# lucidrains/e2-tts-pytorch

Measured on NVIDIA H100. Metric: mel-frames/sec E2TTS fwd+bwd (d512 depth8 L1024), higher is better.
Workload: dtype bf16

## Files before the change

### e2-tts-pytorch_b200/csrc/gemm.cu

```cuda
#include <stdlib.h>

#include "common.cuh"
#include "ptx.cuh"

namespace b200 {

constexpr int BM = 128;
constexpr int BK = 64;
constexpr int kGemmThreads = 384;
constexpr int A_STAGE_BYTES = BM * BK * 2;
constexpr int kSliceBytes = 64 * 64 * 2;

struct GemmParams {
    int M, N, K;
    int tiles_m, tiles_n, num_work;
    int kb_total, kb_per_split, kb_a1;
    void* D; long long ldd; int d_fp32;
    void* D2; long long ldd2;
    const float* bias;
    const float* colscale; int rows_per_batch;
    const unsigned char* rowmask;
    const void* resid; long long ldr;
    int geglu; float dropout_p; unsigned long long seed;
    const unsigned long long* seed_dev;
    int atomic_out;
    int tma_store;
    int resid_tma;
    const float* glu_mult;
};

constexpr int GLU_GELU = 1, GLU_SILU = 2, GLU_RELU2 = 3;
constexpr int ACT_GELU = 1;

template <int BN, int MH>
struct GemmSmem {
    static constexpr int A_BYTES = MH * A_STAGE_BYTES;
    static constexpr int B_STAGE_BYTES = BN * BK * 2;
    static constexpr int STAGE_BYTES = A_BYTES + B_STAGE_BYTES;
    static constexpr int kStages = (STAGE_BYTES <= 32768) ? 6 : 4;
    static constexpr int TILE_BYTES = kStages * STAGE_BYTES;
    static constexpr int STG_BYTES = 2 * 2 * kSliceBytes;
    static constexpr int BAR_BYTES = 128;
    static_assert((2 * kStages + 4) * 8 <= BAR_BYTES, "GEMM mbarriers exceed their shared-memory slot");
    static constexpr int TOTAL = TILE_BYTES + STG_BYTES + BAR_BYTES + 1024;
    static_assert(TOTAL <= 227 * 1024, "GEMM shared memory exceeds the 227 KB a block may use");
};

__device__ __forceinline__ float2 gelu_erf2(float2 x) {
    const float2 a = make_float2(fabsf(x.x), fabsf(x.y));
    float2 t = ffma2(a, make_float2(-1.9449223600531695e-06f, -1.9449223600531695e-06f), make_float2(6.386057066265494e-05f, 6.386057066265494e-05f));
    t = ffma2(t, a, make_float2(-0.0009488713694736362f, -0.0009488713694736362f));
    t = ffma2(t, a, make_float2(0.008582375012338161f, 0.008582375012338161f));
    t = ffma2(t, a, make_float2(-0.0541183240711689f, -0.0541183240711689f));
    t = ffma2(t, a, make_float2(-0.4582974314689636f, -0.4582974314689636f));
    t = ffma2(t, a, make_float2(-1.1513246297836304f, -1.1513246297836304f));
    t = ffma2(t, a, make_float2(-0.9999869465827942f, -0.9999869465827942f));
    float ex, ey;
    asm("ex2.approx.ftz.f32 %0, %1;" : "=f"(ex) : "f"(t.x));
    asm("ex2.approx.ftz.f32 %0, %1;" : "=f"(ey) : "f"(t.y));
    return ffma2(make_float2(-a.x, -a.y), make_float2(ex, ey), make_float2(fmaxf(x.x, 0.f), fmaxf(x.y, 0.f)));
}

__device__ __forceinline__ float2 silu2(float2 x) {
    const float2 t = fmul2(x, make_float2(-1.4426950408889634f, -1.4426950408889634f));
    float ex, ey;
    asm("ex2.approx.ftz.f32 %0, %1;" : "=f"(ex) : "f"(t.x));
    asm("ex2.approx.ftz.f32 %0, %1;" : "=f"(ey) : "f"(t.y));
    const float2 d = fadd2(make_float2(ex, ey), make_float2(1.f, 1.f));
    return make_float2(__fdividef(x.x, d.x), __fdividef(x.y, d.y));
}

__device__ __forceinline__ float2 relu2_2(float2 x) {
    const float2 r = make_float2(fmaxf(x.x, 0.f), fmaxf(x.y, 0.f));
    return fmul2(r, r);
}

template <int ACT>
__device__ __forceinline__ float2 glu_act2(float2 g) {
    if constexpr (ACT == GLU_GELU) return gelu_erf2(g);
    else if constexpr (ACT == GLU_SILU) return silu2(g);
    else return relu2_2(g);
}

__device__ __forceinline__ uint32_t slice_addr(uint32_t buf, uint32_t toff, uint32_t swz, int i, int jj) {
    return buf + toff + (uint32_t)i * 8 * 128 + (((uint32_t)jj << 4) ^ swz);
}
__device__ __forceinline__ uint32_t slice_acquire(uint8_t* my_stg, uint32_t n, int cw, int t) {
    if (t == 0) bulk_wait_group_read<1>();
    named_bar_sync(1 + cw, 128);
    return smem_u32(my_stg + (n & 1) * kSliceBytes);
}
__device__ __forceinline__ void resid_load(const CUtensorMap* m, uint8_t* my_stg, uint64_t* my_rbar, uint32_t b, int c0, int c1) {
    mbar_arrive_expect_tx(&my_rbar[b], kSliceBytes);
    tma_load_2d(my_stg + b * kSliceBytes, m, &my_rbar[b], c0, c1);
}
__device__ __forceinline__ void slice_store(const CUtensorMap* m, uint8_t* my_stg, uint32_t n, int cw, int t, int c0, int c1) {
    fence_proxy_async();
    named_bar_sync(1 + cw, 128);
    if (t == 0) {
        tma_store_2d(m, my_stg + (n & 1) * kSliceBytes, c0, c1);
        bulk_commit_group();
    }
}

template <int ACT, int BN, int MH>
__device__ __forceinline__ void glu_epilogue(const GemmParams& p, float (&acc)[MH][BN / 2], int tm, int tn, int cw, int wq, int lane) {
    constexpr int BMT = BM * MH;
    const int cq = 2 * (lane & 3);
    const bool do_drop = p.dropout_p > 0.f;
    const float keep_scale = do_drop ? 65536.f / (65536.f - (float)(uint32_t)(p.dropout_p * 65536.f)) : 1.f;
    const uint32_t seedmix = do_drop ? seed_mix32(p.seed + (p.seed_dev ? __ldg(p.seed_dev) : 0ull)) : 0u;
    const uint32_t thr32 = drop_thresh32((uint32_t)(p.dropout_p * 65536.f));
#pragma unroll
    for (int h = 0; h < MH; ++h) {
#pragma unroll
        for (int i = 0; i < 2; ++i) {
            const int row = tm * BMT + (cw * MH + h) * 64 + wq * 16 + (lane >> 2) + 8 * i;
            if (row >= p.M) continue;
#pragma unroll
            for (int sub = 0; sub < BN / 128; ++sub) {
                const int colg = tn * BN + sub * 128;
                if (colg >= p.N) continue;
#pragma unroll
                for (int j = 0; j < 8; ++j) {
                    const int cu = colg + 8 * j + cq;
                    const int hcol = colg / 2 + 8 * j + cq;
                    float2 u = make_float2(acc[h][4 * (sub * 16 + j) + 2 * i], acc[h][4 * (sub * 16 + j) + 2 * i + 1]);
                    float2 g = make_float2(acc[h][4 * (sub * 16 + 8 + j) + 2 * i], acc[h][4 * (sub * 16 + 8 + j) + 2 * i + 1]);
                    if (p.bias) {
                        u = fadd2(u, make_float2(__ldg(p.bias + cu), __ldg(p.bias + cu + 1)));
                        g = fadd2(g, make_float2(__ldg(p.bias + cu + 64), __ldg(p.bias + cu + 65)));
                    }
                    const uint32_t wu = pack_bf16(u.x, u.y), wgt = pack_bf16(g.x, g.y);
                    if (p.D2) {
                        __nv_bfloat16* d2 = reinterpret_cast<__nv_bfloat16*>(p.D2) + (long long)row * p.ldd2 + cu;
                        *reinterpret_cast<uint32_t*>(d2) = wu;
                        *reinterpret_cast<uint32_t*>(d2 + 64) = wgt;
                    }
                    float2 h2 = fmul2(make_float2(bf16_lo(wu), bf16_hi(wu)), glu_act2<ACT>(make_float2(bf16_lo(wgt), bf16_hi(wgt))));
                    if (p.glu_mult) h2 = fmul2(h2, make_float2(__ldg(p.glu_mult + hcol), __ldg(p.glu_mult + hcol + 1)));
                    if (do_drop) {
                        const DropWords hsh = drop_words(seedmix, (uint32_t)(((unsigned long long)row * (unsigned long long)(p.N / 2) + hcol) >> 1));
                        h2 = fmul2(h2, make_float2(hsh.a >= thr32 ? keep_scale : 0.f, hsh.b >= thr32 ? keep_scale : 0.f));
                    }
                    *reinterpret_cast<uint32_t*>(reinterpret_cast<__nv_bfloat16*>(p.D) + (long long)row * p.ldd + hcol) = pack_bf16(h2.x, h2.y);
                }
            }
        }
    }
}


template <bool RESID, int BN, int MH>
__device__ __forceinline__ void store_slices(const GemmParams& p, float (&acc)[MH][BN / 2], const CUtensorMap* tmD, const CUtensorMap* tmR,
                                             uint8_t* my_stg, uint64_t* my_rbar, uint32_t& nslice, int tm, int tn, int cw, int wq, int lane,
                                             int t) {
    const uint32_t swz = (uint32_t)(lane >> 2) << 4;
    const uint32_t toff = (uint32_t)(wq * 16 + (lane >> 2)) * 128 + 4 * (lane & 3);
#pragma unroll
    for (int h = 0; h < MH; ++h) {
        const int rowb = tm * BM * MH + (cw * MH + h) * 64;
#pragma unroll
        for (int s = 0; s < BN / 64; ++s) {
            const int colb = tn * BN + s * 64;
            if (colb >= p.N) break;
            uint32_t buf;
            if constexpr (RESID) {
                buf = smem_u32(my_stg + (nslice & 1) * kSliceBytes);
                mbar_wait(&my_rbar[nslice & 1], (nslice >> 1) & 1);
            } else {
                buf = slice_acquire(my_stg, nslice, cw, t);
            }
#pragma unroll
            for (int i = 0; i < 2; ++i) {
#pragma unroll
                for (int jj = 0; jj < 8; ++jj) {
                    const int j = s * 8 + jj;
                    const uint32_t a = slice_addr(buf, toff, swz, i, jj);
                    float v0 = acc[h][4 * j + 2 * i], v1 = acc[h][4 * j + 2 * i + 1];
                    if constexpr (RESID) {
                        const uint32_t r = ld_shared_u32(a);
                        v0 += bf16_lo(r); v1 += bf16_hi(r);
                    }
                    st_shared_u32(a, pack_bf16(v0, v1));
                }
            }
            slice_store(tmD, my_stg, nslice, cw, t, colb, rowb);
            if constexpr (RESID) {
                const bool more = MH == 1 ? (s + 2 < BN / 64 && colb + 128 < p.N) : (h + 1 < MH && tn * BN + 64 < p.N);
                if (t == 0 && more) {
                    bulk_wait_group_read<0>();
                    resid_load(tmR, my_stg, my_rbar, nslice & 1, MH == 1 ? colb + 128 : colb, MH == 1 ? rowb : rowb + 64);
                }
            }
            ++nslice;
        }
    }
}

__device__ __forceinline__ void store_pair(const GemmParams& p, int row, int col, float v0, float v1) {
    const bool two = col + 1 < p.N;
    if (p.d_fp32) {
        float* dp = reinterpret_cast<float*>(p.D) + (long long)row * p.ldd + col;
        const bool vec = two && (reinterpret_cast<uintptr_t>(dp) & 7) == 0;
        if (p.atomic_out) {
            if (vec) atomicAdd(reinterpret_cast<float2*>(dp), make_float2(v0, v1));
            else { atomicAdd(dp, v0); if (two) atomicAdd(dp + 1, v1); }
        } else {
            if (vec) *reinterpret_cast<float2*>(dp) = make_float2(v0, v1);
            else { dp[0] = v0; if (two) dp[1] = v1; }
        }
    } else {
        __nv_bfloat16* dp = reinterpret_cast<__nv_bfloat16*>(p.D) + (long long)row * p.ldd + col;
        if (two) *reinterpret_cast<uint32_t*>(dp) = pack_bf16(v0, v1);
        else dp[0] = __float2bfloat16_rn(v0);
    }
}

template <int BN, bool A_MN, bool B_MN, int MH, int ACT>
__global__ void __launch_bounds__(kGemmThreads, 1)
gemm_wgmma_kernel(const __grid_constant__ CUtensorMap tmA, const __grid_constant__ CUtensorMap tmA2,
                  const __grid_constant__ CUtensorMap tmB, const __grid_constant__ CUtensorMap tmD,
                  const __grid_constant__ CUtensorMap tmR, const GemmParams p) {
    using S = GemmSmem<BN, MH>;
    constexpr int kStages = S::kStages;
    constexpr int BMT = BM * MH;
    constexpr int NACC = BN / 2;
    extern __shared__ uint8_t smem_raw[];
    uint8_t* smem = smem_raw + ((1024u - (smem_u32(smem_raw) & 1023u)) & 1023u);
    uint8_t* smA = smem;
    uint8_t* smB = smem + kStages * S::A_BYTES;
    uint8_t* stg = smem + S::TILE_BYTES;
    uint64_t* full_bar = reinterpret_cast<uint64_t*>(smem + S::TILE_BYTES + S::STG_BYTES);
    uint64_t* empty_bar = full_bar + kStages;
    uint64_t* resid_bar = empty_bar + kStages;

    const int wg = threadIdx.x >> 7;

    if (threadIdx.x == 0) {
        tma_prefetch_desc(&tmA);
        tma_prefetch_desc(&tmA2);
        tma_prefetch_desc(&tmB);
        if (p.tma_store) tma_prefetch_desc(&tmD);
        if (p.resid_tma) tma_prefetch_desc(&tmR);
        for (int i = 0; i < kStages; ++i) {
            mbar_init(&full_bar[i], 1);
            mbar_init(&empty_bar[i], 2);
        }
        for (int i = 0; i < 4; ++i) mbar_init(&resid_bar[i], 1);
        fence_barrier_init();
    }
    __syncthreads();

    if (wg == 0) {
        regs_dealloc<40>();
        if (threadIdx.x == 0) {
            int stage = 0;
            uint32_t phase = 0;
            for (int w = blockIdx.x; w < p.num_work; w += gridDim.x) {
                const int tm = w % p.tiles_m;
                const int rest = w / p.tiles_m;
                const int tn = rest % p.tiles_n;
                const int sp = rest / p.tiles_n;
                const int kb0 = sp * p.kb_per_split;
                const int kb1 = min(p.kb_total, kb0 + p.kb_per_split);
                const int arow = tm * BMT;
                const int brow = tn * BN;
                for (int kb = kb0; kb < kb1; ++kb) {
                    mbar_wait(&empty_bar[stage], phase ^ 1);
                    mbar_arrive_expect_tx(&full_bar[stage], S::STAGE_BYTES);
                    uint8_t* a_dst = smA + stage * S::A_BYTES;
                    uint8_t* b_dst = smB + stage * S::B_STAGE_BYTES;
                    const CUtensorMap* ma = kb < p.kb_a1 ? &tmA : &tmA2;
                    const int ka = kb < p.kb_a1 ? kb * BK : (kb - p.kb_a1) * BK;
                    if constexpr (!A_MN) {
#pragma unroll
                        for (int h = 0; h < MH; ++h) tma_load_2d(a_dst + h * A_STAGE_BYTES, ma, &full_bar[stage], ka, arow + h * BM);
                    } else {
#pragma unroll
                        for (int i = 0; i < BMT / 64; ++i) tma_load_2d(a_dst + i * (BK * 128), ma, &full_bar[stage], arow + i * 64, ka);
                    }
                    if constexpr (!B_MN) {
#pragma unroll
                        for (int h = 0; h < BN / 128; ++h) tma_load_2d(b_dst + h * (128 * BK * 2), &tmB, &full_bar[stage], kb * BK, brow + h * 128);
                    } else {
#pragma unroll
                        for (int i = 0; i < BN / 64; ++i) tma_load_2d(b_dst + i * (BK * 128), &tmB, &full_bar[stage], brow + i * 64, kb * BK);
                    }
                    if (++stage == kStages) { stage = 0; phase ^= 1; }
                }
            }
        }
        return;
    }

    regs_alloc<232>();
    const int cw = wg - 1;
    const int t = threadIdx.x & 127;
    const int lane = t & 31, wq = t >> 5;
    constexpr uint32_t a_lbo = A_MN ? BK * 128 : 16, b_lbo = B_MN ? BK * 128 : 16;
    constexpr uint32_t a_adv = A_MN ? (16 * 128) >> 4 : (16 * 2) >> 4;
    constexpr uint32_t b_adv = B_MN ? (16 * 128) >> 4 : (16 * 2) >> 4;
    float acc[MH][NACC];
    uint8_t* my_stg = stg + cw * 2 * kSliceBytes;
    uint64_t* my_rbar = resid_bar + cw * 2;
    uint32_t nslice = 0;
    int stage = 0;
    uint32_t phase = 0;
    for (int w = blockIdx.x; w < p.num_work; w += gridDim.x) {
        const int tm = w % p.tiles_m;
        const int rest = w / p.tiles_m;
        const int tn = rest % p.tiles_n;
        const int sp = rest / p.tiles_n;
        const int kb0 = sp * p.kb_per_split;
        const int kb1 = min(p.kb_total, kb0 + p.kb_per_split);
        const int kb_resid = max(kb0, kb1 - 2);
        int prev = -1;
        for (int kb = kb0; kb < kb1; ++kb) {
            mbar_wait(&full_bar[stage], phase);
#pragma unroll
            for (int h = 0; h < MH; ++h) fence_regs(acc[h]);
            wgmma_fence();
            const uint64_t bdesc = make_smem_desc_sw128(smem_u32(smB + stage * S::B_STAGE_BYTES), b_lbo, 1024);
#pragma unroll
            for (int h = 0; h < MH; ++h) {
                const uint64_t adesc = make_smem_desc_sw128(smem_u32(smA + stage * S::A_BYTES + (cw * MH + h) * 8192), a_lbo, 1024);
#pragma unroll
                for (int k = 0; k < BK / 16; ++k) {
                    const uint32_t accum = (kb > kb0 || k > 0) ? 1u : 0u;
                    if constexpr (BN == 256) wgmma_ss_n256<A_MN, B_MN>(acc[h], adesc + (uint64_t)(k * a_adv), bdesc + (uint64_t)(k * b_adv), accum);
                    else wgmma_ss_n128<A_MN, B_MN>(acc[h], adesc + (uint64_t)(k * a_adv), bdesc + (uint64_t)(k * b_adv), accum);
                }
            }
            wgmma_commit();
            if (p.resid_tma && kb == kb_resid && t == 0) {
                const int r0 = tm * BMT + cw * MH * 64;
                bulk_wait_group_read<0>();
                resid_load(&tmR, my_stg, my_rbar, nslice & 1, tn * BN, r0);
                if (tn * BN + 64 < p.N) resid_load(&tmR, my_stg, my_rbar, (nslice + 1) & 1, tn * BN + 64, r0);
                else if (MH == 2) resid_load(&tmR, my_stg, my_rbar, (nslice + 1) & 1, tn * BN, r0 + 64);
            }
            wgmma_wait<1>();
#pragma unroll
            for (int h = 0; h < MH; ++h) fence_regs(acc[h]);
            if (prev >= 0 && t == 0) mbar_arrive(&empty_bar[prev]);
            prev = stage;
            if (++stage == kStages) { stage = 0; phase ^= 1; }
        }
        wgmma_wait<0>();
#pragma unroll
        for (int h = 0; h < MH; ++h) fence_regs(acc[h]);
        if (prev >= 0 && t == 0) mbar_arrive(&empty_bar[prev]);

        const int cq = 2 * (lane & 3);
        if (p.tma_store) {
            const bool resid_ldg = p.resid && !p.resid_tma;
            if (ACT || p.bias || p.colscale || p.rowmask || resid_ldg) {
#pragma unroll
                for (int h = 0; h < MH; ++h) {
#pragma unroll
                    for (int i = 0; i < 2; ++i) {
                        const int row = tm * BMT + (cw * MH + h) * 64 + wq * 16 + (lane >> 2) + 8 * i;
                        if (row >= p.M) continue;
                        const bool masked = p.rowmask && p.rowmask[row] == 0;
                        const float* cs = p.colscale ? p.colscale + (long long)(row / p.rows_per_batch) * p.N : nullptr;
                        const __nv_bfloat16* rp = resid_ldg ? reinterpret_cast<const __nv_bfloat16*>(p.resid) + (long long)row * p.ldr : nullptr;
#pragma unroll
                        for (int j = 0; j < BN / 8; ++j) {
                            const int col = tn * BN + 8 * j + cq;
                            if (col >= p.N) continue;
                            const bool two = col + 1 < p.N;
                            float v0 = acc[h][4 * j + 2 * i], v1 = acc[h][4 * j + 2 * i + 1];
                            if (p.bias) { v0 += __ldg(p.bias + col); if (two) v1 += __ldg(p.bias + col + 1); }
                            if constexpr (ACT == ACT_GELU) { const float2 g = gelu_erf2(make_float2(v0, v1)); v0 = g.x; v1 = g.y; }
                            if (cs) { v0 *= __ldg(cs + col); if (two) v1 *= __ldg(cs + col + 1); }
                            if (masked) { v0 = 0.f; v1 = 0.f; }
                            if (rp) {
                                if (two) {
                                    const uint32_t u = *reinterpret_cast<const uint32_t*>(rp + col);
                                    v0 += bf16_lo(u); v1 += bf16_hi(u);
                                } else {
                                    v0 += __bfloat162float(rp[col]);
                                }
                            }
                            acc[h][4 * j + 2 * i] = v0;
                            acc[h][4 * j + 2 * i + 1] = v1;
                        }
                    }
                }
            }
            if (p.resid_tma) store_slices<true, BN, MH>(p, acc, &tmD, &tmR, my_stg, my_rbar, nslice, tm, tn, cw, wq, lane, t);
            else store_slices<false, BN, MH>(p, acc, &tmD, &tmR, my_stg, my_rbar, nslice, tm, tn, cw, wq, lane, t);
        } else if (!p.geglu) {
#pragma unroll
            for (int h = 0; h < MH; ++h) {
#pragma unroll
                for (int i = 0; i < 2; ++i) {
                    const int row = tm * BMT + (cw * MH + h) * 64 + wq * 16 + (lane >> 2) + 8 * i;
                    if (row >= p.M) continue;
                    const bool masked = p.rowmask && p.rowmask[row] == 0;
                    const float* cs = p.colscale ? p.colscale + (long long)(row / p.rows_per_batch) * p.N : nullptr;
                    const __nv_bfloat16* rp = p.resid ? reinterpret_cast<const __nv_bfloat16*>(p.resid) + (long long)row * p.ldr : nullptr;
#pragma unroll
                    for (int j = 0; j < BN / 8; ++j) {
                        const int col = tn * BN + 8 * j + cq;
                        if (col >= p.N) continue;
                        const bool two = col + 1 < p.N;
                        float v0 = acc[h][4 * j + 2 * i], v1 = acc[h][4 * j + 2 * i + 1];
                        if (p.bias) { v0 += __ldg(p.bias + col); if (two) v1 += __ldg(p.bias + col + 1); }
                        if constexpr (ACT == ACT_GELU) { const float2 g = gelu_erf2(make_float2(v0, v1)); v0 = g.x; v1 = g.y; }
                        if (cs) { v0 *= __ldg(cs + col); if (two) v1 *= __ldg(cs + col + 1); }
                        if (masked) { v0 = 0.f; v1 = 0.f; }
                        if (rp) {
                            if (two) {
                                const uint32_t u = *reinterpret_cast<const uint32_t*>(rp + col);
                                v0 += bf16_lo(u); v1 += bf16_hi(u);
                            } else {
                                v0 += __bfloat162float(rp[col]);
                            }
                        }
                        store_pair(p, row, col, v0, v1);
                    }
                }
            }
        } else if (p.geglu == GLU_GELU) {
            glu_epilogue<GLU_GELU, BN, MH>(p, acc, tm, tn, cw, wq, lane);
        } else if (p.geglu == GLU_SILU) {
            glu_epilogue<GLU_SILU, BN, MH>(p, acc, tm, tn, cw, wq, lane);
        } else {
            glu_epilogue<GLU_RELU2, BN, MH>(p, acc, tm, tn, cw, wq, lane);
        }
    }
    if (t == 0) bulk_wait_group<0>();
}


typedef CUresult (*PFN_encodeTiled)(CUtensorMap*, CUtensorMapDataType, cuuint32_t, void*, const cuuint64_t*, const cuuint64_t*,
                                    const cuuint32_t*, const cuuint32_t*, CUtensorMapInterleave, CUtensorMapSwizzle,
                                    CUtensorMapL2promotion, CUtensorMapFloatOOBfill);

static PFN_encodeTiled get_encode_fn() {
    static PFN_encodeTiled fn = nullptr;
    if (!fn) {
        void* ptr = nullptr;
        cudaDriverEntryPointQueryResult qres;
        if (cudaGetDriverEntryPoint("cuTensorMapEncodeTiled", &ptr, cudaEnableDefault, &qres) == cudaSuccess &&
            qres == cudaDriverEntryPointSuccess)
            fn = reinterpret_cast<PFN_encodeTiled>(ptr);
    }
    return fn;
}

struct MapKey { const void* ptr; int64_t inner, outer, ld; int box, box_inner; };
struct MapSlot { MapKey k; CUtensorMap m; bool valid; };
static int make_map_uncached(CUtensorMap* m, const void* ptr, int64_t inner, int64_t outer, int64_t ld, int box_outer, int box_inner);
static int make_map(CUtensorMap* m, const void* ptr, int64_t inner, int64_t outer, int64_t ld, int box_outer, int box_inner = 64) {
    constexpr int kSlots = 1024;
    static thread_local MapSlot cache[kSlots];
    uint64_t h = reinterpret_cast<uintptr_t>(ptr) >> 4;
    h = (h ^ (uint64_t)inner * 0x9E3779B97F4A7C15ull ^ (uint64_t)outer * 0xC2B2AE3D27D4EB4Full ^ (uint64_t)ld * 0x165667B19E3779F9ull ^ (uint64_t)(box_outer * 131 + box_inner)) * 0xFF51AFD7ED558CCDull;
    MapSlot& sl = cache[(h >> 40) % kSlots];
    if (sl.valid && sl.k.ptr == ptr && sl.k.inner == inner && sl.k.outer == outer && sl.k.ld == ld && sl.k.box == box_outer && sl.k.box_inner == box_inner) {
        *m = sl.m;
        return 0;
    }
    if (int rc = make_map_uncached(m, ptr, inner, outer, ld, box_outer, box_inner)) return rc;
    sl.k = MapKey{ptr, inner, outer, ld, box_outer, box_inner};
    sl.m = *m;
    sl.valid = true;
    return 0;
}
static int make_map_uncached(CUtensorMap* m, const void* ptr, int64_t inner, int64_t outer, int64_t ld, int box_outer, int box_inner) {
    PFN_encodeTiled enc = get_encode_fn();
    B200_REQUIRE(enc, "cuTensorMapEncodeTiled entry point not available");
    B200_REQUIRE((ld % 8) == 0, "gemm: row pitch %lld not a multiple of 8 elements", (long long)ld);
    B200_REQUIRE((reinterpret_cast<uintptr_t>(ptr) & 15) == 0, "gemm: operand not 16-byte aligned");
    cuuint64_t gdim[2] = {(cuuint64_t)inner, (cuuint64_t)outer};
    cuuint64_t gstride[1] = {(cuuint64_t)ld * 2};
    cuuint32_t box[2] = {(cuuint32_t)box_inner, (cuuint32_t)box_outer};
    cuuint32_t estr[2] = {1, 1};
    CUresult r = enc(m, CU_TENSOR_MAP_DATA_TYPE_BFLOAT16, 2, const_cast<void*>(ptr), gdim, gstride, box, estr,
                     CU_TENSOR_MAP_INTERLEAVE_NONE, box_inner == 64 ? CU_TENSOR_MAP_SWIZZLE_128B : CU_TENSOR_MAP_SWIZZLE_64B,
                     CU_TENSOR_MAP_L2_PROMOTION_L2_256B, CU_TENSOR_MAP_FLOAT_OOB_FILL_NONE);
    B200_REQUIRE(r == CUDA_SUCCESS, "cuTensorMapEncodeTiled failed (%d)", (int)r);
    return 0;
}

template <int BN, bool A_MN, bool B_MN, int MH, int ACT = 0>
static int launch_gemm(const CUtensorMap (&tm)[5], const GemmParams& p, cudaStream_t st) {
    using S = GemmSmem<BN, MH>;
    auto kern = gemm_wgmma_kernel<BN, A_MN, B_MN, MH, ACT>;
    static DeviceOnce once;
    {
        cudaError_t e = set_max_smem_once(once, kern, S::TOTAL);
        B200_REQUIRE(e == cudaSuccess, "gemm: cudaFuncSetAttribute: %s", cudaGetErrorString(e));
    }
    const int grid = p.num_work < num_sms() ? p.num_work : num_sms();
    kern<<<grid, kGemmThreads, S::TOTAL, st>>>(tm[0], tm[1], tm[2], tm[3], tm[4], p);
    return check_launch("gemm_wgmma_kernel");
}

}

using namespace b200;

extern "C" int b200_gemm(const b200_gemm_args* a, b200_stream_t stream) {
    cudaStream_t st = reinterpret_cast<cudaStream_t>(stream);
    B200_REQUIRE(a && a->A && a->B && a->D, "gemm: null operand");
    B200_REQUIRE(a->M > 0 && a->N > 0 && a->K > 0, "gemm: empty problem %lldx%lldx%lld", (long long)a->M, (long long)a->N, (long long)a->K);
    B200_REQUIRE(a->M < (1ll << 31) && a->N < (1ll << 31) && a->K < (1ll << 31), "gemm: dimension too large");
    const bool a_mn = a->a_mn_major != 0, b_mn = a->b_mn_major != 0;
    GemmParams p{};
    p.M = (int)a->M; p.N = (int)a->N; p.K = (int)a->K;
    const bool wide = a->force_tile == 3 || (a->force_tile == 0 && p.M >= 512 && p.N >= 256);
    const int BN = wide ? 256 : 128;
    const int MH = wide ? 1 : (a->force_tile == 1) ? 1 : ((a->force_tile == 2 || p.M >= 256) ? 2 : 1);
    const int tile_rows = BM * MH;
    p.tiles_m = (p.M + tile_rows - 1) / tile_rows;
    p.tiles_n = (p.N + BN - 1) / BN;
    p.kb_total = (p.K + BK - 1) / BK;
    p.kb_a1 = p.kb_total;
    if (a->A2) {
        B200_REQUIRE(a->K1 > 0 && a->K1 < a->K && (a->K1 % BK) == 0, "gemm: K1=%lld must be a multiple of %d inside (0,K)", (long long)a->K1, BK);
        p.kb_a1 = (int)(a->K1 / BK);
    }
    int split = a->split_k > 1 ? a->split_k : 1;
    if (a->split_k < 0) {
        const int units = num_sms();
        const int tiles = p.tiles_m * p.tiles_n;
        int s_fill = (units + tiles / 2) / tiles;
        while (s_fill > 1 && tiles * s_fill > units) --s_fill;
        const int s_max = p.kb_total / 8;
        split = s_fill < 1 ? 1 : s_fill;
        if (split > s_max) split = s_max < 1 ? 1 : s_max;
        if (split > 64) split = 64;
    }
    if (split > p.kb_total) split = p.kb_total;
    p.kb_per_split = (p.kb_total + split - 1) / split;
    split = (p.kb_total + p.kb_per_split - 1) / p.kb_per_split;
    p.num_work = p.tiles_m * p.tiles_n * split;
    p.atomic_out = split > 1;
    p.D = a->D; p.ldd = a->ldd; p.d_fp32 = a->d_fp32;
    p.D2 = a->D2; p.ldd2 = a->ldd2;
    p.bias = a->bias; p.colscale = a->colscale; p.rows_per_batch = (int)(a->rows_per_batch > 0 ? a->rows_per_batch : 1);
    p.rowmask = a->rowmask; p.resid = a->resid; p.ldr = a->ldr;
    B200_REQUIRE(a->geglu >= 0 && a->geglu <= GLU_RELU2, "gemm: geglu=%d is not an activation code (0 none, 1 GELU, 2 SiLU, 3 ReLU^2)", (int)a->geglu);
    B200_REQUIRE(!a->glu_mult || a->geglu, "gemm: glu_mult needs the GLU epilogue (geglu != 0)");
    p.geglu = a->geglu; p.dropout_p = a->dropout_p; p.seed = a->seed; p.seed_dev = reinterpret_cast<const unsigned long long*>(a->seed_dev);
    p.glu_mult = a->glu_mult;
    if (p.atomic_out) {
        B200_REQUIRE(a->d_fp32, "gemm: split-K requires an fp32 output");
        B200_REQUIRE(!a->bias && !a->colscale && !a->rowmask && !a->resid && !a->geglu, "gemm: split-K supports no epilogue");
        cudaError_t e = cudaMemset2DAsync(a->D, (size_t)a->ldd * 4, 0, (size_t)a->N * 4, (size_t)a->M, st);
        B200_REQUIRE(e == cudaSuccess, "gemm: memset: %s", cudaGetErrorString(e));
    }
    if (a->geglu) {
        B200_REQUIRE((a->N % 128) == 0 && !a->d_fp32 && !a->colscale && !a->rowmask && !a->resid, "gemm: GEGLU needs N %% 128 == 0, bf16 out, no other epilogue");
        B200_REQUIRE((a->ldd % 8) == 0 && (!a->D2 || (a->ldd2 % 8) == 0), "gemm: GEGLU output pitch must be a multiple of 8");
        B200_REQUIRE(!a->bias || (reinterpret_cast<uintptr_t>(a->bias) & 15) == 0, "gemm: GEGLU bias must be 16-byte aligned");
    }
    B200_REQUIRE(a->act == 0 || a->act == ACT_GELU, "gemm: act=%d is not an activation code (0 none, 1 GELU)", (int)a->act);
    if (a->act) {
        B200_REQUIRE(!a->geglu && a->split_k >= 0 && a->split_k <= 1 && !a->d_fp32, "gemm: act needs a bf16 output without GLU or split-K");
        B200_REQUIRE(!a_mn && !b_mn, "gemm: act is built for K-major operands only");
        B200_REQUIRE((reinterpret_cast<uintptr_t>(a->D) & 15) == 0, "gemm: act needs a 16-byte aligned output (TMA tile stores)");
    }
    if (!a->d_fp32) B200_REQUIRE((a->ldd % 8) == 0, "gemm: bf16 output pitch must be a multiple of 8");
    if (a->resid) B200_REQUIRE((a->ldr % 8) == 0, "gemm: residual pitch must be a multiple of 8");

    CUtensorMap tm[5];
    CUtensorMap &tA = tm[0], &tA2 = tm[1], &tB = tm[2], &tD = tm[3], &tR = tm[4];
    int rc;
    const int64_t KA = a->A2 ? a->K1 : a->K;
    if (!a_mn) rc = make_map(&tA, a->A, KA, a->M, a->lda, BM);
    else rc = make_map(&tA, a->A, a->M, a->K, a->lda, BK);
    if (rc) return rc;
    if (a->A2) {
        if (!a_mn) rc = make_map(&tA2, a->A2, a->K - a->K1, a->M, a->lda2, BM);
        else rc = make_map(&tA2, a->A2, a->M, a->K - a->K1, a->lda2, BK);
        if (rc) return rc;
    } else {
        tA2 = tA;
    }
    if (!b_mn) rc = make_map(&tB, a->B, a->K, a->N, a->ldb, 128);
    else rc = make_map(&tB, a->B, a->N, a->K, a->ldb, BK);
    if (rc) return rc;
    if (!a->d_fp32) B200_REQUIRE((reinterpret_cast<uintptr_t>(a->D) & 3) == 0, "gemm: bf16 output must be 4-byte aligned");
    const auto a16 = [](const void* q) { return (reinterpret_cast<uintptr_t>(q) & 15) == 0; };
    p.tma_store = !a->d_fp32 && !a->geglu && a16(a->D) && (p.N % 8) == 0;
    p.resid_tma = p.tma_store && a->resid && a16(a->resid);
    tD = tR = tB;
    if (p.tma_store && (rc = make_map(&tD, a->D, a->N, a->M, a->ldd, 64))) return rc;
    if (p.resid_tma && (rc = make_map(&tR, a->resid, a->N, a->M, a->ldr, 64))) return rc;
    if (a->geglu && a->D2) B200_REQUIRE((reinterpret_cast<uintptr_t>(a->D2) & 3) == 0, "gemm: GEGLU pre-activation buffer must be 4-byte aligned");
    if (a->resid) B200_REQUIRE((reinterpret_cast<uintptr_t>(a->resid) & 3) == 0, "gemm: residual must be 4-byte aligned");

    {
        static const bool trace = getenv("B200_GEMM_TRACE") != nullptr;
        if (trace)
            fprintf(stderr, "GEMMTRACE %d %d %d amn=%d bmn=%d split=%d geglu=%d two=%d mh=%d epi=%d%d%d%d\n", p.M, p.N, p.K, (int)a_mn, (int)b_mn, split,
                    p.geglu, a->A2 != nullptr, wide ? 3 : MH, p.bias != nullptr, p.colscale != nullptr, p.rowmask != nullptr, p.resid != nullptr);
    }
    if (a->act) {
        if (wide) return launch_gemm<256, false, false, 1, ACT_GELU>(tm, p, st);
        if (MH == 2) return launch_gemm<128, false, false, 2, ACT_GELU>(tm, p, st);
        return launch_gemm<128, false, false, 1, ACT_GELU>(tm, p, st);
    }
    if (wide) {
        if (!a_mn && !b_mn) return launch_gemm<256, false, false, 1>(tm, p, st);
        if (!a_mn && b_mn) return launch_gemm<256, false, true, 1>(tm, p, st);
        if (a_mn && !b_mn) return launch_gemm<256, true, false, 1>(tm, p, st);
        return launch_gemm<256, true, true, 1>(tm, p, st);
    }
    if (MH == 2) {
        if (!a_mn && !b_mn) return launch_gemm<128, false, false, 2>(tm, p, st);
        if (!a_mn && b_mn) return launch_gemm<128, false, true, 2>(tm, p, st);
        if (a_mn && !b_mn) return launch_gemm<128, true, false, 2>(tm, p, st);
        return launch_gemm<128, true, true, 2>(tm, p, st);
    }
    if (!a_mn && !b_mn) return launch_gemm<128, false, false, 1>(tm, p, st);
    if (!a_mn && b_mn) return launch_gemm<128, false, true, 1>(tm, p, st);
    if (a_mn && !b_mn) return launch_gemm<128, true, false, 1>(tm, p, st);
    return launch_gemm<128, true, true, 1>(tm, p, st);
}
```

Baseline: 335,500.

## Route GEGLU epilogue through swizzled smem slices with TMA stores and bulk-loaded bias

Adds a TMA-based epilogue for GLU GEMMs. The pre-activation tile is staged in swizzled shared-memory slices and written with TMA. The gated product is then computed from those staged slices and stored through a second tensor map. Bias and GLU multiplier vectors are bulk-loaded into shared memory by the producer thread, with their own full/empty mbarrier pair per tile, replacing per-fragment global stores and loads. This adds shared memory, barriers and extra named-barrier syncs, and only applies to K-major operands with aligned buffers.

```diff
diff --git a/e2-tts-pytorch_b200/csrc/gemm.cu b/e2-tts-pytorch_b200/csrc/gemm.cu
--- a/e2-tts-pytorch_b200/csrc/gemm.cu
+++ b/e2-tts-pytorch_b200/csrc/gemm.cu
@@ -27,6 +27,7 @@
     int tma_store;
     int resid_tma;
     const float* glu_mult;
+    int glu_tma;
 };
 
 constexpr int GLU_GELU = 1, GLU_SILU = 2, GLU_RELU2 = 3;
@@ -40,9 +41,10 @@
     static constexpr int kStages = (STAGE_BYTES <= 32768) ? 6 : 4;
     static constexpr int TILE_BYTES = kStages * STAGE_BYTES;
     static constexpr int STG_BYTES = 2 * 2 * kSliceBytes;
-    static constexpr int BAR_BYTES = 128;
-    static_assert((2 * kStages + 4) * 8 <= BAR_BYTES, "GEMM mbarriers exceed their shared-memory slot");
-    static constexpr int TOTAL = TILE_BYTES + STG_BYTES + BAR_BYTES + 1024;
+    static constexpr int BAR_BYTES = 256;
+    static_assert((2 * kStages + 4 + 2) * 8 <= BAR_BYTES, "GEMM mbarriers exceed their shared-memory slot");
+    static constexpr int OPS_BYTES = BN * 4 + BN / 2 * 4;
+    static constexpr int TOTAL = TILE_BYTES + STG_BYTES + BAR_BYTES + OPS_BYTES + 1024;
     static_assert(TOTAL <= 227 * 1024, "GEMM shared memory exceeds the 227 KB a block may use");
 };
 
@@ -85,6 +87,11 @@
 __device__ __forceinline__ uint32_t slice_addr(uint32_t buf, uint32_t toff, uint32_t swz, int i, int jj) {
     return buf + toff + (uint32_t)i * 8 * 128 + (((uint32_t)jj << 4) ^ swz);
 }
+__device__ __forceinline__ uint32_t slice_toff(int wq) {
+    uint32_t l;
+    asm volatile("mov.u32 %0, %%laneid;" : "=r"(l));
+    return (uint32_t)(wq * 16 + (l >> 2)) * 128 + 4 * (l & 3);
+}
 __device__ __forceinline__ uint32_t slice_acquire(uint8_t* my_stg, uint32_t n, int cw, int t) {
     if (t == 0) bulk_wait_group_read<1>();
     named_bar_sync(1 + cw, 128);
@@ -193,6 +200,66 @@
                     resid_load(tmR, my_stg, my_rbar, nslice & 1, MH == 1 ? colb + 128 : colb, MH == 1 ? rowb : rowb + 64);
                 }
             }
+            ++nslice;
+        }
+    }
+}
+
+template <int ACT, int BN, int MH>
+__device__ __forceinline__ void glu_store_slices(const GemmParams& p, float (&acc)[MH][BN / 2], const CUtensorMap* tmD, const CUtensorMap* tmD2,
+                                                 uint8_t* my_stg, const float* sbias, const float* smult, uint32_t& nslice, int tm, int tn,
+                                                 int cw, int wq, int lane, int t) {
+    const uint32_t swz = (uint32_t)(lane >> 2) << 4;
+    const uint32_t toff = slice_toff(wq);
+    const int cq = 2 * (lane & 3);
+    const bool do_drop = p.dropout_p > 0.f;
+    const float keep_scale = do_drop ? 65536.f / (65536.f - (float)(uint32_t)(p.dropout_p * 65536.f)) : 1.f;
+    const uint32_t seedmix = do_drop ? seed_mix32(p.seed + (p.seed_dev ? __ldg(p.seed_dev) : 0ull)) : 0u;
+    const uint32_t thr32 = drop_thresh32((uint32_t)(p.dropout_p * 65536.f));
+#pragma unroll
+    for (int h = 0; h < MH; ++h) {
+        const int rowb = tm * BM * MH + (cw * MH + h) * 64;
+#pragma unroll
+        for (int sub = 0; sub < BN / 128; ++sub) {
+            const int colg = tn * BN + sub * 128;
+            if (colg >= p.N) break;
+#pragma unroll
+            for (int half = 0; half < 2; ++half) {
+                const uint32_t buf = slice_acquire(my_stg, nslice, cw, t);
+#pragma unroll
+                for (int i = 0; i < 2; ++i) {
+#pragma unroll
+                    for (int jj = 0; jj < 8; ++jj) {
+                        const int j = sub * 16 + half * 8 + jj;
+                        float2 v = make_float2(acc[h][4 * j + 2 * i], acc[h][4 * j + 2 * i + 1]);
+                        if (p.bias) v = fadd2(v, *reinterpret_cast<const float2*>(sbias + 8 * j + cq));
+                        st_shared_u32(slice_addr(buf, toff, swz, i, jj), pack_bf16(v.x, v.y));
+                    }
+                }
+                slice_store(tmD2, my_stg, nslice, cw, t, colg + 64 * half, rowb);
+                ++nslice;
+            }
+            const uint32_t bu = slice_acquire(my_stg, nslice, cw, t);
+            const uint32_t bg = smem_u32(my_stg + ((nslice + 1) & 1) * kSliceBytes);
+#pragma unroll
+            for (int i = 0; i < 2; ++i) {
+                const int row = rowb + wq * 16 + (lane >> 2) + 8 * i;
+#pragma unroll
+                for (int jj = 0; jj < 8; ++jj) {
+                    const int hl = sub * 64 + 8 * jj + cq;
+                    const uint32_t a = slice_addr(bu, toff, swz, i, jj);
+                    const uint32_t wu = ld_shared_u32(a), wgt = ld_shared_u32(slice_addr(bg, toff, swz, i, jj));
+                    float2 h2 = fmul2(make_float2(bf16_lo(wu), bf16_hi(wu)), glu_act2<ACT>(make_float2(bf16_lo(wgt), bf16_hi(wgt))));
+                    if (p.glu_mult) h2 = fmul2(h2, *reinterpret_cast<const float2*>(smult + hl));
+                    if (do_drop) {
+                        const int hcol = tn * (BN / 2) + hl;
+                        const DropWords hsh = drop_words(seedmix, (uint32_t)(((unsigned long long)row * (unsigned long long)(p.N / 2) + hcol) >> 1));
+                        h2 = fmul2(h2, make_float2(hsh.a >= thr32 ? keep_scale : 0.f, hsh.b >= thr32 ? keep_scale : 0.f));
+                    }
+                    st_shared_u32(a, pack_bf16(h2.x, h2.y));
+                }
+            }
+            slice_store(tmD, my_stg, nslice, cw, t, colg / 2, rowb);
             ++nslice;
         }
     }
@@ -221,7 +288,7 @@
 __global__ void __launch_bounds__(kGemmThreads, 1)
 gemm_wgmma_kernel(const __grid_constant__ CUtensorMap tmA, const __grid_constant__ CUtensorMap tmA2,
                   const __grid_constant__ CUtensorMap tmB, const __grid_constant__ CUtensorMap tmD,
-                  const __grid_constant__ CUtensorMap tmR, const GemmParams p) {
+                  const __grid_constant__ CUtensorMap tmR, const __grid_constant__ CUtensorMap tmD2, const GemmParams p) {
     using S = GemmSmem<BN, MH>;
     constexpr int kStages = S::kStages;
     constexpr int BMT = BM * MH;
@@ -234,6 +301,11 @@
     uint64_t* full_bar = reinterpret_cast<uint64_t*>(smem + S::TILE_BYTES + S::STG_BYTES);
     uint64_t* empty_bar = full_bar + kStages;
     uint64_t* resid_bar = empty_bar + kStages;
+    uint64_t* ops_full = resid_bar + 4;
+    uint64_t* ops_empty = ops_full + 1;
+    float* sops = reinterpret_cast<float*>(smem + S::TILE_BYTES + S::STG_BYTES + S::BAR_BYTES);
+    constexpr bool kGluTma = !A_MN && !B_MN;
+    const bool glu_ops = kGluTma && p.glu_tma && (p.bias || p.glu_mult);
 
     const int wg = threadIdx.x >> 7;
 
@@ -243,11 +315,17 @@
         tma_prefetch_desc(&tmB);
         if (p.tma_store) tma_prefetch_desc(&tmD);
         if (p.resid_tma) tma_prefetch_desc(&tmR);
+        if (kGluTma && p.glu_tma) {
+            tma_prefetch_desc(&tmD);
+            tma_prefetch_desc(&tmD2);
+        }
         for (int i = 0; i < kStages; ++i) {
             mbar_init(&full_bar[i], 1);
             mbar_init(&empty_bar[i], 2);
         }
         for (int i = 0; i < 4; ++i) mbar_init(&resid_bar[i], 1);
+        mbar_init(ops_full, 1);
+        mbar_init(ops_empty, 2);
         fence_barrier_init();
     }
     __syncthreads();
@@ -257,7 +335,8 @@
         if (threadIdx.x == 0) {
             int stage = 0;
             uint32_t phase = 0;
-            for (int w = blockIdx.x; w < p.num_work; w += gridDim.x) {
+            uint32_t ntile = 0;
+            for (int w = blockIdx.x; w < p.num_work; w += gridDim.x, ++ntile) {
                 const int tm = w % p.tiles_m;
                 const int rest = w / p.tiles_m;
                 const int tn = rest % p.tiles_n;
@@ -289,6 +368,13 @@
                     }
                     if (++stage == kStages) { stage = 0; phase ^= 1; }
                 }
+                if (glu_ops) {
+                    const int nb = min(BN, p.N - brow);
+                    mbar_wait(ops_empty, (ntile & 1) ^ 1);
+                    mbar_arrive_expect_tx(ops_full, (p.bias ? nb * 4 : 0) + (p.glu_mult ? nb * 2 : 0));
+                    if (p.bias) bulk_load_1d(sops, p.bias + brow, nb * 4, ops_full);
+                    if (p.glu_mult) bulk_load_1d(sops + BN, p.glu_mult + brow / 2, nb * 2, ops_full);
+                }
             }
         }
         return;
@@ -307,7 +393,8 @@
     uint32_t nslice = 0;
     int stage = 0;
     uint32_t phase = 0;
-    for (int w = blockIdx.x; w < p.num_work; w += gridDim.x) {
+    uint32_t ntile = 0;
+    for (int w = blockIdx.x; w < p.num_work; w += gridDim.x, ++ntile) {
         const int tm = w % p.tiles_m;
         const int rest = w / p.tiles_m;
         const int tn = rest % p.tiles_n;
@@ -391,6 +478,14 @@
             }
             if (p.resid_tma) store_slices<true, BN, MH>(p, acc, &tmD, &tmR, my_stg, my_rbar, nslice, tm, tn, cw, wq, lane, t);
             else store_slices<false, BN, MH>(p, acc, &tmD, &tmR, my_stg, my_rbar, nslice, tm, tn, cw, wq, lane, t);
+        } else if (kGluTma && p.glu_tma) {
+            if constexpr (kGluTma) {
+                if (glu_ops) mbar_wait(ops_full, ntile & 1);
+                if (p.geglu == GLU_GELU) glu_store_slices<GLU_GELU, BN, MH>(p, acc, &tmD, &tmD2, my_stg, sops, sops + BN, nslice, tm, tn, cw, wq, lane, t);
+                else if (p.geglu == GLU_SILU) glu_store_slices<GLU_SILU, BN, MH>(p, acc, &tmD, &tmD2, my_stg, sops, sops + BN, nslice, tm, tn, cw, wq, lane, t);
+                else glu_store_slices<GLU_RELU2, BN, MH>(p, acc, &tmD, &tmD2, my_stg, sops, sops + BN, nslice, tm, tn, cw, wq, lane, t);
+                if (glu_ops && t == 0) mbar_arrive(ops_empty);
+            }
         } else if (!p.geglu) {
 #pragma unroll
             for (int h = 0; h < MH; ++h) {
@@ -487,7 +582,7 @@
 }
 
 template <int BN, bool A_MN, bool B_MN, int MH, int ACT = 0>
-static int launch_gemm(const CUtensorMap (&tm)[5], const GemmParams& p, cudaStream_t st) {
+static int launch_gemm(const CUtensorMap (&tm)[6], const GemmParams& p, cudaStream_t st) {
     using S = GemmSmem<BN, MH>;
     auto kern = gemm_wgmma_kernel<BN, A_MN, B_MN, MH, ACT>;
     static DeviceOnce once;
@@ -496,7 +591,7 @@
         B200_REQUIRE(e == cudaSuccess, "gemm: cudaFuncSetAttribute: %s", cudaGetErrorString(e));
     }
     const int grid = p.num_work < num_sms() ? p.num_work : num_sms();
-    kern<<<grid, kGemmThreads, S::TOTAL, st>>>(tm[0], tm[1], tm[2], tm[3], tm[4], p);
+    kern<<<grid, kGemmThreads, S::TOTAL, st>>>(tm[0], tm[1], tm[2], tm[3], tm[4], tm[5], p);
     return check_launch("gemm_wgmma_kernel");
 }
 
@@ -568,8 +663,8 @@
     if (!a->d_fp32) B200_REQUIRE((a->ldd % 8) == 0, "gemm: bf16 output pitch must be a multiple of 8");
     if (a->resid) B200_REQUIRE((a->ldr % 8) == 0, "gemm: residual pitch must be a multiple of 8");
 
-    CUtensorMap tm[5];
-    CUtensorMap &tA = tm[0], &tA2 = tm[1], &tB = tm[2], &tD = tm[3], &tR = tm[4];
+    CUtensorMap tm[6];
+    CUtensorMap &tA = tm[0], &tA2 = tm[1], &tB = tm[2], &tD = tm[3], &tR = tm[4], &tD2 = tm[5];
     int rc;
     const int64_t KA = a->A2 ? a->K1 : a->K;
     if (!a_mn) rc = make_map(&tA, a->A, KA, a->M, a->lda, BM);
@@ -589,17 +684,21 @@
     const auto a16 = [](const void* q) { return (reinterpret_cast<uintptr_t>(q) & 15) == 0; };
     p.tma_store = !a->d_fp32 && !a->geglu && a16(a->D) && (p.N % 8) == 0;
     p.resid_tma = p.tma_store && a->resid && a16(a->resid);
-    tD = tR = tB;
+    p.glu_tma = a->geglu && !a_mn && !b_mn && a->D2 && a16(a->D) && a16(a->D2) && (!a->glu_mult || a16(a->glu_mult));
+    tD = tR = tD2 = tB;
     if (p.tma_store && (rc = make_map(&tD, a->D, a->N, a->M, a->ldd, 64))) return rc;
     if (p.resid_tma && (rc = make_map(&tR, a->resid, a->N, a->M, a->ldr, 64))) return rc;
+    if (p.glu_tma && (rc = make_map(&tD, a->D, a->N / 2, a->M, a->ldd, 64))) return rc;
+    if (p.glu_tma && (rc = make_map(&tD2, a->D2, a->N, a->M, a->ldd2, 64))) return rc;
     if (a->geglu && a->D2) B200_REQUIRE((reinterpret_cast<uintptr_t>(a->D2) & 3) == 0, "gemm: GEGLU pre-activation buffer must be 4-byte aligned");
     if (a->resid) B200_REQUIRE((reinterpret_cast<uintptr_t>(a->resid) & 3) == 0, "gemm: residual must be 4-byte aligned");
 
     {
         static const bool trace = getenv("B200_GEMM_TRACE") != nullptr;
         if (trace)
-            fprintf(stderr, "GEMMTRACE %d %d %d amn=%d bmn=%d split=%d geglu=%d two=%d mh=%d epi=%d%d%d%d\n", p.M, p.N, p.K, (int)a_mn, (int)b_mn, split,
-                    p.geglu, a->A2 != nullptr, wide ? 3 : MH, p.bias != nullptr, p.colscale != nullptr, p.rowmask != nullptr, p.resid != nullptr);
+            fprintf(stderr, "GEMMTRACE %d %d %d amn=%d bmn=%d split=%d geglu=%d two=%d mh=%d epi=%d%d%d%d store=%s\n", p.M, p.N, p.K, (int)a_mn,
+                    (int)b_mn, split, p.geglu, a->A2 != nullptr, wide ? 3 : MH, p.bias != nullptr, p.colscale != nullptr, p.rowmask != nullptr,
+                    p.resid != nullptr, (p.tma_store || p.glu_tma) ? "tma" : "frag");
     }
     if (a->act) {
         if (wide) return launch_gemm<256, false, false, 1, ACT_GELU>(tm, p, st);
```

New measurement: 348,300, median of 6. +3.8%, better.
